# scanner-research/scannertools

Measured on AMD Instinct MI355X. Metric: 1080p frames/sec (optical-flow + histogram ops), higher is better.
Workload: dtype f32 (u8 frames in; the box filter's running sums in f64, re-anchored every 32 rows / 8 columns, column sums handed to the row pass as f32)

## Files before the change

scannertools_amd/csrc/st_context.hip:

```cpp
#include <cstring>
#include <vector>
#include <mutex>
#include <chrono>
#include <cstdlib>

#include "st_internal.h"

int st_set_error(st_ctx* ctx, int status, const char* fmt, ...) {
  char buf[512];
  va_list ap;
  va_start(ap, fmt);
  vsnprintf(buf, sizeof(buf), fmt, ap);
  va_end(ap);
  if (ctx) ctx->last_error = buf;
  return status;
}

int st_enter(st_ctx* ctx) {
  if (!ctx) return ST_ERR_INVALID;
  ST_HIP(ctx, hipSetDevice(ctx->device));
  return ST_OK;
}

namespace {
// ... 52 lines not shown
}

ST_EXPORT int st_device_count(int* count) {
  if (!count) return ST_ERR_INVALID;
  int n = 0;
  hipError_t e = hipGetDeviceCount(&n);
  if (e != hipSuccess) { *count = 0; return ST_ERR_HIP; }
  *count = n;
  return ST_OK;
}

static constexpr size_t kMinLdsBytes = 160 * 1024;

ST_EXPORT int st_ctx_create(int device_id, st_ctx** out_ctx) {
  if (!out_ctx) return ST_ERR_INVALID;
  *out_ctx = nullptr;
  int n = 0;
  if (hipGetDeviceCount(&n) != hipSuccess || device_id < 0 || device_id >= n) return ST_ERR_INVALID;
  if (hipSetDevice(device_id) != hipSuccess) return ST_ERR_HIP;
  st_ctx* c = new (std::nothrow) st_ctx();
  if (!c) return ST_ERR_OOM;
  c->device = device_id;
  if (hipStreamCreateWithFlags(&c->own_stream, hipStreamNonBlocking) != hipSuccess) {
    delete c;
    return ST_ERR_HIP;
  }
  c->stream = c->own_stream;
  if (const char* e = getenv("ST_ITER_TILE")) c->tile_mode = atoi(e);
  c->fold_gray = getenv("ST_PYR_FOLD_GRAY") != nullptr;
  if (const char* e = getenv("ST_POLY_U8")) c->poly_u8 = atoi(e) != 0;
  if (const char* e = getenv("ST_ITER_ROLES")) c->roles_mode = atoi(e);
  if (const char* e = getenv("ST_ROLES_NCW")) c->roles_ncw = atoi(e);
  if (const char* e = getenv("ST_PYR_ROLES")) c->pyr_roles = atoi(e);
  if (const char* e = getenv("ST_CONV_TILE")) c->conv_tile = atoi(e);
  if (const char* e = getenv("ST_CONCURRENT")) c->concurrency_mode = atoi(e);
  hipDeviceProp_t prop;
  if (hipGetDeviceProperties(&prop, device_id) == hipSuccess) {
    c->num_cus = prop.multiProcessorCount;
    if (prop.sharedMemPerBlock < kMinLdsBytes || strncmp(prop.gcnArchName, "gfx950", 6) != 0) {
      (void)hipStreamDestroy(c->own_stream);
      delete c;
      return ST_ERR_UNSUPPORTED;
    }
  }
  reg_add(c);
  *out_ctx = c;
  return ST_OK;
}

ST_EXPORT int st_ctx_destroy(st_ctx* ctx) {
  if (!ctx) return ST_ERR_INVALID;
  reg_remove(ctx);
  (void)hipSetDevice(ctx->device);
  (void)hipStreamSynchronize(ctx->stream);
  for (auto& t : ctx->timing) {
    for (auto e : t.starts) (void)hipEventDestroy(e);
    for (auto e : t.stops) (void)hipEventDestroy(e);
  }
  if (ctx->ws) (void)hipFree(ctx->ws);
  st_jpeg_release(ctx);
  st_netin_release(ctx);
  st_detect_release(ctx);
  if (ctx->own_stream) (void)hipStreamDestroy(ctx->own_stream);
  delete ctx;
  return ST_OK;
}
// ... 175 lines not shown
```

scannertools_amd/csrc/st_farneback.hip:

```cpp
#include <cmath>
#include <cstdlib>
#include <cstring>

#include "st_internal.h"

namespace {

constexpr int kMaxTaps = 32;
constexpr int kMaxPolyN = 7;

inline int cv_round(double v) { return (int)lrint(v); }

struct LevelGeom {
  int lh, lw, ksize;
  double sigma, scale;
};

int fb_levels(int h, int w, const st_fb_params& p) {
  int k;
  double scale = 1;
  for (k = 0; k < p.num_levels; ++k) {
    scale *= p.pyr_scale;
    if (w * scale < 32 || h * scale < 32) break;
  }
  return k;
}

LevelGeom fb_level_geom(int h, int w, const st_fb_params& p, int k) {
  LevelGeom g;
  double scale = 1;
  for (int i = 0; i < k; ++i) scale *= p.pyr_scale;
  g.scale = scale;
// ... 461 lines not shown
  float hA[KS + 1], hB[KS + 1];
#pragma unroll
  for (int j = 0; j <= KS; ++j) hA[j] = hB[j] = 0.f;
  const int ys0 = S * dy0 + OFF - r;
  const int nsrc = KS + 1 + S * (dy1 - dy0 - 1);
  int dy = dy0, until = KS + 1;
#pragma unroll 1
  for (int t = 0; t < nsrc; ++t) {
    float nA, nB;
    hrow(ys0 + t, nA, nB);
#pragma unroll
    for (int j = 0; j < KS; ++j) { hA[j] = hA[j + 1]; hB[j] = hB[j + 1]; }
    hA[KS] = nA; hB[KS] = nB;
    if (t + 1 == until) {
      until += S;
      const float b00 = pyr_colfilter<KS>(hA, a.taps), b01 = pyr_colfilter<KS>(hB, a.taps);
      const float b10 = pyr_colfilter<KS>(hA + 1, a.taps), b11 = pyr_colfilter<KS>(hB + 1, a.taps);
      float out;
      if (S == 2) {
        out = ((b00 + b01) + (b10 + b11)) * 0.25f;
      } else {
        const float r0 = b00 * 0.5f + b01 * 0.5f, r1 = b10 * 0.5f + b11 * 0.5f;
        out = r0 * 0.5f + r1 * 0.5f;
      }
      dst[(size_t)dy * a.dw + dx] = out;
      ++dy;
    }
  }
}

struct PyrFusedArgs {
  const uint8_t* gray;
  const uint8_t* const* frames;
  int cb, cg, cr, rnd, shift;
  float* img0; float* img1; float* img2; float* img3;
  int h, w, rows_per_seg;
  int strip_w;
  float k0[2], k1[2], k2[5], k3[10];
};

template <int KS>
__device__ __forceinline__ float pf_rowfilter(const float* __restrict__ b, const float* __restrict__ kh) {
  constexpr int r = KS / 2;
  if (KS == 3) return b[1] * kh[1] + (b[0] + b[2]) * kh[0];
  float v = kh[0] * b[0];
#pragma unroll
  for (int i = 1; i < KS; ++i) v += kh[i <= r ? i : KS - 1 - i] * b[i];
  return v;
}
template <int KS>
__device__ __forceinline__ float pf_colfilter(const float* __restrict__ c, const float* __restrict__ kh) {
  constexpr int r = KS / 2;
  if (KS == 3) return (c[0] + c[2]) * kh[0] + c[1] * kh[1];
  float s = kh[r] * c[r];
#pragma unroll
  for (int i = 1; i <= r; ++i) s += kh[r - i] * (c[r + i] + c[r - i]);
  return s;
}

constexpr int PF_RB = 8;
constexpr int PF_ROWDW = 260;

__device__ __forceinline__ unsigned pf_load4_border(const uint8_t* __restrict__ row, int col0, int w) {
  unsigned v = 0;
#pragma unroll 1
  for (int k = 0; k < 4; ++k) v |= (unsigned)row[d_reflect101(col0 + k, w)] << (8 * k);
// ... 154 lines not shown
        unsigned dw[6];
#pragma unroll
        for (int q = 0; q < 6; ++q) dw[q] = s[2 * u + q];
        float cb[21];
#pragma unroll
        for (int q = 0; q < 6; ++q) {
          const unsigned d = __builtin_amdgcn_alignbyte(dw[q + 1 < 6 ? q + 1 : 5], dw[q], (unsigned)half);
#pragma unroll
          for (int k = 0; k < 4; ++k)
            if (4 * q + k < 21) cb[4 * q + k] = pf_byte(d, k);
        }
        const float n3 = pf_rowfilter<19>(cb + 2, a.k3);
#pragma unroll
        for (int j = 0; j < 19; ++j) r3[j] = r3[j + 1];
        r3[19] = n3;
        if (r == 5) {
          const int dy = (y - 13) >> 3;
          if (dy >= (Y0 >> 3) && dy < (Y1 >> 3)) {
            const float c0 = pf_colfilter<19>(r3, a.k3), c1 = pf_colfilter<19>(r3 + 1, a.k3);
            const float p0 = __shfl_xor(c0, 32), p1 = __shfl_xor(c1, 32);
            if (half == 0 && live3) {
              const float q0 = c0 * 0.5f + p0 * 0.5f, q1 = c1 * 0.5f + p1 * 0.5f;
              o3[(size_t)dy * (w >> 3) + (X0 >> 3) + u] = q0 * 0.5f + q1 * 0.5f;
            }
          }
        }
      }
    }
    if (b + 1 < nb) stash(buf ^ 1);
    __syncthreads();
  }
}

template <int ROLE, bool L0 = true>
__device__ __forceinline__ void pyr_role_run(const PyrFusedArgs& a, unsigned (*srow)[PF_RB][PF_ROWDW]) {
  const int t = threadIdx.x & 255, lane = t & 63, wv = t >> 6;
  const int h = a.h, w = a.w;
  const int SW = a.strip_w;
  const int X0 = blockIdx.x * SW;
  const int Y0 = blockIdx.y * a.rows_per_seg, Y1 = min(h, Y0 + a.rows_per_seg);
  const size_t np = (size_t)h * w;
  const uint8_t* __restrict__ g = a.gray + (size_t)blockIdx.z * np;
  float* __restrict__ o0 = a.img0 + (size_t)blockIdx.z * np;
  float* __restrict__ o1 = a.img1 + (size_t)blockIdx.z * (np >> 2);
  float* __restrict__ o2 = a.img2 + (size_t)blockIdx.z * (np >> 4);
  float* __restrict__ o3 = a.img3 + (size_t)blockIdx.z * (np >> 6);
  const int u = wv * 32 + (lane & 31), half = lane >> 5;
  const bool live = 4 * t < SW && X0 + 4 * t < w;
  const bool live3 = 8 * u < SW && X0 + 8 * u < w;
  const int hq = t & 3, hrow = (t >> 2) & 7;
  const int hcol = hq < 2 ? X0 - 8 + 4 * hq : X0 + SW + 4 * (hq - 2);
  const int hidx = hq < 2 ? hq : 2 + (SW >> 2) + (hq - 2);

  unsigned pre[3], preh = 0u;
  auto fetch = [&](int ybase) {
#pragma unroll
    for (int j = 0; j < 3; ++j) {
      const int r = ROLE + 3 * j;
      if (r < PF_RB) pre[j] = pf_load4(g + (size_t)d_reflect101(ybase + r, h) * w, X0 + 4 * t, w);
    }
    if (ROLE == 0 && t < 32) preh = pf_load4(g + (size_t)d_reflect101(ybase + hrow, h) * w, hcol, w);
  };
  auto stash = [&](int buf) {
    if (4 * t < SW) {
#pragma unroll
      for (int j = 0; j < 3; ++j) {
        const int r = ROLE + 3 * j;
        if (r < PF_RB) srow[buf][r][2 + t] = pre[j];
      }
    }
    if (ROLE == 0 && t < 32) srow[buf][hrow][hidx] = preh;
  };

  float hm[4], hc[4], r1A[2][4], r1B[2][4];
  float r2A[10], r2B[10];
  float r3[20];
  if (ROLE == 0) {
#pragma unroll
    for (int j = 0; j < 4; ++j) { hm[j] = hc[j] = 0.f; r1A[0][j] = r1A[1][j] = r1B[0][j] = r1B[1][j] = 0.f; }
  } else if (ROLE == 1) {
#pragma unroll
    for (int j = 0; j < 10; ++j) r2A[j] = r2B[j] = 0.f;
  } else {
#pragma unroll
    for (int j = 0; j < 20; ++j) r3[j] = 0.f;
  }

  const int nb = (Y1 - Y0) / PF_RB + 2;
  fetch(Y0 - PF_RB);
  stash(0);
  __syncthreads();
  for (int b = 0; b < nb; ++b) {
    const int ybase = Y0 - PF_RB + b * PF_RB;
    const int buf = b & 1;
    if (b + 1 < nb) fetch(ybase + PF_RB);
#pragma unroll
    for (int r = 0; r < PF_RB; ++r) {
      const int y = ybase + r;
      const unsigned* __restrict__ s = srow[buf][r];
      if (ROLE == 0) {
        const unsigned d0 = s[t + 1], d1 = s[t + 2], d2 = s[t + 3];
        float bb[12];
#pragma unroll
        for (int k = 0; k < 4; ++k) { bb[k] = pf_byte(d0, k); bb[4 + k] = pf_byte(d1, k); bb[8 + k] = pf_byte(d2, k); }
        if (L0) {
          float hp[4];
#pragma unroll
          for (int j = 0; j < 4; ++j) hp[j] = bb[4 + j] * a.k0[1] + (bb[3 + j] + bb[5 + j]) * a.k0[0];
          const int yo = y - 1;
          if (live && yo >= Y0 && yo < Y1) {
            float4 v;
            v.x = (hm[0] + hp[0]) * a.k0[0] + hc[0] * a.k0[1];
            v.y = (hm[1] + hp[1]) * a.k0[0] + hc[1] * a.k0[1];
            v.z = (hm[2] + hp[2]) * a.k0[0] + hc[2] * a.k0[1];
            v.w = (hm[3] + hp[3]) * a.k0[0] + hc[3] * a.k0[1];
            *reinterpret_cast<float4*>(o0 + (size_t)yo * w + X0 + 4 * t) = v;
          }
#pragma unroll
          for (int j = 0; j < 4; ++j) { hm[j] = hc[j]; hc[j] = hp[j]; }
        }
        {
#pragma unroll
          for (int e = 0; e < 2; ++e) {
// ... 37 lines not shown
            const float q0 = b00 * 0.5f + b01 * 0.5f, q1 = b10 * 0.5f + b11 * 0.5f;
            o2[(size_t)dy * (w >> 2) + (X0 >> 2) + t] = q0 * 0.5f + q1 * 0.5f;
          }
        }
      } else {
        unsigned dw[6];
#pragma unroll
        for (int q = 0; q < 6; ++q) dw[q] = s[2 * u + q];
        float cb[21];
#pragma unroll
        for (int q = 0; q < 6; ++q) {
          const unsigned d = __builtin_amdgcn_alignbyte(dw[q + 1 < 6 ? q + 1 : 5], dw[q], (unsigned)half);
#pragma unroll
          for (int k = 0; k < 4; ++k)
            if (4 * q + k < 21) cb[4 * q + k] = pf_byte(d, k);
        }
        const float n3 = pf_rowfilter<19>(cb + 2, a.k3);
#pragma unroll
        for (int j = 0; j < 19; ++j) r3[j] = r3[j + 1];
        r3[19] = n3;
        if (r == 5) {
          const int dy = (y - 13) >> 3;
          if (dy >= (Y0 >> 3) && dy < (Y1 >> 3)) {
            const float c0 = pf_colfilter<19>(r3, a.k3), c1 = pf_colfilter<19>(r3 + 1, a.k3);
            const float p0 = __shfl_xor(c0, 32), p1 = __shfl_xor(c1, 32);
            if (half == 0 && live3) {
              const float q0 = c0 * 0.5f + p0 * 0.5f, q1 = c1 * 0.5f + p1 * 0.5f;
              o3[(size_t)dy * (w >> 3) + (X0 >> 3) + u] = q0 * 0.5f + q1 * 0.5f;
            }
          }
        }
      }
    }
    if (b + 1 < nb) stash(buf ^ 1);
    __syncthreads();
  }
}

template <bool L0>
__global__ __launch_bounds__(768) void k_pyr_roles(PyrFusedArgs a) {
  __shared__ unsigned srow[2][PF_RB][PF_ROWDW];
  const int role = threadIdx.x >> 8;
  if (role == 0) pyr_role_run<0, L0>(a, srow);
  else if (role == 1) pyr_role_run<1>(a, srow);
  else pyr_role_run<2>(a, srow);
}

typedef float f2u __attribute__((ext_vector_type(2), aligned(4)));
typedef float f4v16 __attribute__((ext_vector_type(4)));
__device__ __forceinline__ __amdgpu_buffer_rsrc_t st_rsrc(const void* base, size_t bytes) {
  return __builtin_amdgcn_make_buffer_rsrc(const_cast<void*>(base), 0, (int)(bytes > 0xfffffffcull ? 0xfffffffcull : bytes), 0x00020000);
}
__device__ __forceinline__ float bld1(__amdgpu_buffer_rsrc_t r, unsigned voff, unsigned soff) {
  return __builtin_bit_cast(float, __builtin_amdgcn_raw_buffer_load_b32(r, (int)voff, (int)soff, 0));
}
template <int AUX = 0>
__device__ __forceinline__ void bst1(__amdgpu_buffer_rsrc_t r, unsigned voff, unsigned soff, float v) {
  __builtin_amdgcn_raw_buffer_store_b32(__builtin_bit_cast(unsigned, v), r, (int)voff, (int)soff, AUX);
}
template <int AUX = 0>
__device__ __forceinline__ void bst4(__amdgpu_buffer_rsrc_t r, unsigned voff, float4 v) {
  typedef unsigned u4 __attribute__((ext_vector_type(4)));
  u4 q;
  q.x = __builtin_bit_cast(unsigned, v.x); q.y = __builtin_bit_cast(unsigned, v.y);
  q.z = __builtin_bit_cast(unsigned, v.z); q.w = __builtin_bit_cast(unsigned, v.w);
  __builtin_amdgcn_raw_buffer_store_b128(q, r, (int)voff, 0, AUX);
}

__device__ __forceinline__ float ldf(const float* __restrict__ base, unsigned byte_off) {
  return *reinterpret_cast<const float*>(reinterpret_cast<const char*>(base) + byte_off);
}
__device__ __forceinline__ f2u ldf2(const float* __restrict__ base, unsigned byte_off) {
  return *reinterpret_cast<const f2u*>(reinterpret_cast<const char*>(base) + byte_off);
}
__device__ __forceinline__ float4 ldf4(const float* __restrict__ base, unsigned byte_off) {
  return *reinterpret_cast<const float4*>(reinterpret_cast<const char*>(base) + byte_off);
}

// ... 832 lines not shown
  const unsigned C = gx * gy, N = C * gz;
  if (N % 8u) return;
  const unsigned L = bx + gx * (by + gy * bz), xcd = L % 8u, slot = L / 8u;
  unsigned col, pair;
  if (C % 8u == 0) {
    const unsigned cpx = C / 8u;
    col = xcd + 8u * (slot % cpx);
    pair = slot / cpx;
  } else if (8u % C == 0 && gz % (8u / C) == 0) {
    col = xcd % C;
    pair = (xcd / C) * (gz / (8u / C)) + slot;
  } else {
    return;
  }
  bx = col % gx; by = col / gx; bz = pair;
}

template <int MODE>
__global__ __launch_bounds__(B2_T, 2) void k_flow_iter3(IterArgs a) {
  typedef float f2v __attribute__((ext_vector_type(2)));
  constexpr int M = 7, W = 2 * M + 1, RB = 2;
  static_assert(W == F3_RING - 1 && F3_GROUP % RB == 0 && M <= B2_HALO, "ring of 16 = window of 15 + the entering row");
  __shared__ float Vs[F3_GROUP][5][F3_PADW];
  __shared__ float2 Fs[F3_GROUP][F3_PADW];
  const int tid = threadIdx.x;
  const int h = a.h, w = a.w;
  const int np = h * w;
  unsigned bx = blockIdx.x, by = blockIdx.y, bz = blockIdx.z;
  xcd_remap(bx, by, bz);
  const int pr = bz;
  const int x = (int)bx * B2_OUT - B2_HALO + tid;
  const int xc = d_clamp(x, 0, w - 1);
  const int y0 = by * a.rows_per_seg;
  const int y1 = min(h, y0 + a.rows_per_seg);
  const bool writer = tid >= B2_HALO && tid < B2_T - B2_HALO && x < w;
  const int vpos = f3_pos(tid);
  typedef float f4v __attribute__((ext_vector_type(4), aligned(8)));
  const bool pair_tid = tid >= B2_HALO && tid < B2_T - B2_HALO;
  const int pair_k = pair_tid ? tid - B2_HALO : 0, pair_j = pair_k % (B2_OUT / 2);
  const int pair_r0 = (pair_k / (B2_OUT / 2)) * (F3_GROUP / 2);
  const int pair_x = (int)bx * B2_OUT + 2 * pair_j;
  const int pair_pos = f3_pos(B2_HALO + 2 * pair_j);

  const float* __restrict__ R0;
  const float* __restrict__ R1;
  if (a.pairs) {
    R0 = a.R + (size_t)a.pairs[2 * pr] * 5 * (size_t)np;
    R1 = a.R + (size_t)a.pairs[2 * pr + 1] * 5 * (size_t)np;
  } else {
    R0 = a.R;
    R1 = a.R1_direct;
  }
  const float* __restrict__ fin = a.flow_in ? a.flow_in + (size_t)pr * 2 * (size_t)np : nullptr;
  const float* __restrict__ C = a.coarse ? a.coarse + (size_t)pr * 2 * (size_t)a.ch * a.cw : nullptr;
  float* fout = a.flow_ptrs ? st_gl(a.flow_ptrs[pr]) : a.flow_out + (size_t)pr * 2 * (size_t)np;
  const CoarseX cx = (MODE == FLOW_COARSE || MODE == FLOW_COARSE2) ? coarse_x(a, xc) : CoarseX{0, 1.f, 0.f, false};

  float ring[F3_RING][5];
#pragma unroll
  for (int s0 = 0; s0 < W; s0 += 3) {
    UmLoads Li[3];
    float2 f[3];
#pragma unroll
    for (int i = 0; i < 3; ++i) {
      const int yy = d_clamp(y0 - M + s0 + i, 0, h - 1);
      f[i] = iter_flow_at<MODE>(a, fin, C, cx, xc, yy);
      um_issue(R0, R1, np, h, w, xc, yy, f[i], Li[i]);
// ... 696 lines not shown
    int rows = (int)((g.lh + segs - 1) / segs);
    const int min_rows = S == 8 ? 4 : 8;
    if (rows < min_rows) rows = g.lh < min_rows ? g.lh : min_rows;
    z.rows_per_seg = rows;
    dim3 grid(bx, (g.lh + rows - 1) / rows, n);
    st_timed t(ctx, ST_K_PYR);
    if (S == 2) hipLaunchKernelGGL((k_pyr_dec<2, 3>), grid, dim3(256), 0, ctx->stream, z);
    else if (S == 4) hipLaunchKernelGGL((k_pyr_dec<4, 9>), grid, dim3(256), 0, ctx->stream, z);
    else hipLaunchKernelGGL((k_pyr_dec<8, 19>), grid, dim3(256), 0, ctx->stream, z);
    ST_HIP(ctx, hipGetLastError());
    return ST_OK;
  }
  a.mode = q.mode; a.max_rows = q.max_rows; a.max_cols = q.max_cols;
  const size_t lds = q.lds;
  if (lds > kPyrLdsMax) return st_set_error(ctx, ST_ERR_UNSUPPORTED, "farneback: pyramid tile needs %zu B of LDS", lds);
  dim3 grid((g.lw + PYR_OW - 1) / PYR_OW, (g.lh + PYR_OH - 1) / PYR_OH, n);
  st_timed t(ctx, ST_K_PYR);
  hipLaunchKernelGGL(k_pyr, grid, dim3(256), lds, ctx->stream, a);
  ST_HIP(ctx, hipGetLastError());
  return ST_OK;
}

bool pyr_fused_ok(int h, int w, const st_fb_params& p) {
  if (fb_levels(h, w, p) != 3 || (h & 7) || (w & 7)) return false;
  static const int ks[4] = {3, 3, 9, 19};
  for (int k = 0; k <= 3; ++k) {
    const LevelGeom g = fb_level_geom(h, w, p, k);
    if (g.lh != (h >> k) || g.lw != (w >> k) || g.ksize != ks[k]) return false;
  }
  return true;
}

int launch_pyr_fused(st_ctx* ctx, const uint8_t* gray, const uint8_t* const* frames, int n, int h, int w,
                     const st_fb_params& p, float* const imgs[4], bool skip0 = false) {
  PyrFusedArgs a;
  memset(&a, 0, sizeof(a));
  a.gray = gray; a.frames = frames;
  if (p.gray_bits == 14) { a.cb = 1868; a.cg = 9617; a.cr = 4899; } else { a.cb = 3735; a.cg = 19235; a.cr = 9798; }
  a.shift = p.gray_bits; a.rnd = 1 << (p.gray_bits - 1);
  a.img0 = imgs[0]; a.img1 = imgs[1]; a.img2 = imgs[2]; a.img3 = imgs[3];
  a.h = h; a.w = w;
  float* taps[4] = {a.k0, a.k1, a.k2, a.k3};
  for (int k = 0; k <= 3; ++k) {
    const LevelGeom g = fb_level_geom(h, w, p, k);
    float full[kMaxTaps];
    gaussian_kernel(g.ksize, g.sigma, full);
    for (int i = 0; i <= g.ksize / 2; ++i) {
      if (full[i] != full[g.ksize - 1 - i]) return st_set_error(ctx, ST_ERR_UNSUPPORTED, "pyr: asymmetric Gaussian taps");
      taps[k][i] = full[i];
    }
  }
  const int strips = (w + 1023) / 1024;
  a.strip_w = ((w + strips - 1) / strips + 7) / 8 * 8;
  const bool roles_on = gray && ctx->pyr_roles != 0;
  long long segs = ((long long)ctx->num_cus * (roles_on ? 14 : 8) + (long long)strips * n - 1) / ((long long)strips * n);
  int rows = (int)((h + segs - 1) / segs);
  rows = (rows + 7) / 8 * 8;
  const int min_rows = (long long)strips * n * ((h + 63) / 64) >= 2LL * ctx->num_cus ? 64 : 16;
  if (rows < min_rows) rows = h < min_rows ? h : min_rows;
  a.rows_per_seg = rows;
  st_timed t(ctx, ST_K_PYR);
  const int roles_env = ctx->pyr_roles;
  const bool roles = gray && roles_env != 0;
  if (skip0 && !roles) return st_set_error(ctx, ST_ERR_INVALID, "pyr: level 0 can only be left out of the role-split kernel");
  if (roles && skip0) hipLaunchKernelGGL(k_pyr_roles<false>, dim3(strips, (h + rows - 1) / rows, n), dim3(768), 0, ctx->stream, a);
  else if (roles) hipLaunchKernelGGL(k_pyr_roles<true>, dim3(strips, (h + rows - 1) / rows, n), dim3(768), 0, ctx->stream, a);
  else if (gray) hipLaunchKernelGGL(k_pyr_fused<false>, dim3(strips, (h + rows - 1) / rows, n), dim3(256), 0, ctx->stream, a);
  else hipLaunchKernelGGL(k_pyr_fused<true>, dim3(strips, (h + rows - 1) / rows, n), dim3(256), 0, ctx->stream, a);
  ST_HIP(ctx, hipGetLastError());
  return ST_OK;
}

static bool polyexp_frame_fits(int h, int w) { return (unsigned long long)h * (unsigned long long)w <= (1ull << 26); }

int launch_polyexp(st_ctx* ctx, const float* img, int n, int h, int w, int poly_n, double poly_sigma, float* R,
                   const uint8_t* gray = nullptr) {
  if (!polyexp_frame_fits(h, w)) return st_set_error(ctx, ST_ERR_UNSUPPORTED, "polyexp: frames above 64 M pixels are not supported");
  PolyArgs a;
  a.img = img; a.gray = gray; a.R = R; a.h = h; a.w = w;
  poly_prepare(poly_n, poly_sigma, &a.c);
  const int strips = (w + PE_OUT - 1) / PE_OUT;
  a.rows_per_seg = polyexp_rows(ctx, h, strips, n, poly_n);
  dim3 grid(strips, (h + a.rows_per_seg - 1) / a.rows_per_seg, n);
  st_timed t(ctx, ST_K_POLYEXP);
  if (gray && w < 8) return st_set_error(ctx, ST_ERR_INVALID, "polyexp: the gray-source instance needs rows of at least 8 pixels");
  if (gray && poly_n == 5) hipLaunchKernelGGL(k_polyexp_u8<5>, grid, dim3(256), 0, ctx->stream, a);
  else if (gray) hipLaunchKernelGGL(k_polyexp_u8<7>, grid, dim3(256), 0, ctx->stream, a);
  else if (poly_n == 5) hipLaunchKernelGGL(k_polyexp<5>, grid, dim3(256), 0, ctx->stream, a);
  else hipLaunchKernelGGL(k_polyexp<7>, grid, dim3(256), 0, ctx->stream, a);
  ST_HIP(ctx, hipGetLastError());
  return ST_OK;
}

int launch_polyexp_ml(st_ctx* ctx, float* const* imgs, const LevelGeom* geom, float* const* R, const int* ks, int nk, int n,
                      int poly_n, double poly_sigma) {
  if (nk < 1 || nk > 4) return st_set_error(ctx, ST_ERR_INVALID, "polyexp: bad level list");
  PolyArgsML a;
  memset(&a, 0, sizeof(a));
// ... 22 lines not shown
  int bx = (int)((np + 255) / 256);
  if (bx > 4096) bx = 4096;
  st_timed t(ctx, ST_K_UPDATE_MATRICES);
  hipLaunchKernelGGL(k_update_matrices, dim3(bx, n_pairs), dim3(256), 0, ctx->stream, a);
  ST_HIP(ctx, hipGetLastError());
  return ST_OK;
}

int launch_blur(st_ctx* ctx, BlurArgs a, int n_pairs) {
  if (a.m == 7) {
    const int strips = (a.w + B2_OUT - 1) / B2_OUT;
    long long segs = ((long long)ctx->num_cus * 4 + (long long)strips - 1) / ((long long)strips);
    int rows = (int)((a.h + segs - 1) / segs);
    rows = (rows + 14) / 15 * 15;
    if (rows < 15) rows = 15;
    if (rows > 135 && a.h > 135) rows = 135;
    a.rows_per_seg = rows;
    dim3 grid(strips, (a.h + rows - 1) / rows, n_pairs);
    st_timed t(ctx, ST_K_BLUR_UPDATE);
    hipLaunchKernelGGL((k_blur_update_v2<7>), grid, dim3(B2_T), 0, ctx->stream, a);
    ST_HIP(ctx, hipGetLastError());
    return ST_OK;
  }
  const int strips = (a.w + (BLUR_T - 2 * a.m) - 1) / (BLUR_T - 2 * a.m);
  a.rows_per_seg = rows_per_segment(ctx, a.h, strips, 1, 2 * a.m + 1);
  dim3 grid(strips, (a.h + a.rows_per_seg - 1) / a.rows_per_seg, n_pairs);
  st_timed t(ctx, ST_K_BLUR_UPDATE);
  hipLaunchKernelGGL(k_blur_update, grid, dim3(BLUR_T), 0, ctx->stream, a);
  ST_HIP(ctx, hipGetLastError());
  return ST_OK;
}

int launch_flow_iter(st_ctx* ctx, IterArgs a, int n_pairs) {
  constexpr long long kTilePx = 600000;
  const bool tile = ctx->tile_mode == 1 || (ctx->tile_mode != 0 && (long long)n_pairs * a.h * a.w <= kTilePx);
  if (tile && (a.h + FT_T - 1) / FT_T <= 65535) {
    dim3 grid((a.w + FT_T - 1) / FT_T, (a.h + FT_T - 1) / FT_T, n_pairs);
    st_timed t(ctx, ST_K_BLUR_UPDATE);
    if (a.coarse) hipLaunchKernelGGL((k_flow_iter_tile<FLOW_COARSE>), grid, dim3(FT_NT), 0, ctx->stream, a);
    else if (a.flow_in) hipLaunchKernelGGL((k_flow_iter_tile<FLOW_FIELD>), grid, dim3(FT_NT), 0, ctx->stream, a);
    else hipLaunchKernelGGL((k_flow_iter_tile<FLOW_ZERO>), grid, dim3(FT_NT), 0, ctx->stream, a);
    ST_HIP(ctx, hipGetLastError());
    return ST_OK;
  }
  const int strips = (a.w + B2_OUT - 1) / B2_OUT;
  const long long resident = (long long)ctx->num_cus * 2;
  const int periods = (a.h + F3_ANCHOR - 1) / F3_ANCHOR;
  int rows = periods * F3_ANCHOR;
  long long rounds3 = 1, wgs3 = 1;
  double best = 1e300;
  for (int segs = 1; segs <= periods; ++segs) {
    const int r = (periods + segs - 1) / segs * F3_ANCHOR;
    const long long nseg = (a.h + r - 1) / r;
    const long long wgs = (long long)strips * n_pairs * nseg;
    const long long rounds = (wgs + resident - 1) / resident;
    const double cost = (double)rounds * (r + 15);
    if (cost < best * 0.999) { best = cost; rows = r; rounds3 = rounds; wgs3 = wgs; }
  }
  const int roles_env = ctx->roles_mode == -1 && ctx->flow_concurrent ? 0 : ctx->roles_mode;
  const int roles_ncw = ctx->roles_ncw;
  const long long roles_limit = a.coarse ? resident * 62 / 100 : resident * 95 / 100;
  if (roles_env == 1 || (roles_env != 0 && rounds3 == 1 && wgs3 < roles_limit)) {
    int best_ncw = 0, best_out = 0, best_rows = 0;
    double bestr = 1e300;
    for (int ncw = 5; ncw >= 4; --ncw) {
      if (roles_ncw && ncw != roles_ncw) continue;
      const int outmax = 64 * ncw - 2 * B2_HALO;
      const int rstrips = (a.w + outmax - 1) / outmax;
      const int out_w = ((a.w + rstrips - 1) / rstrips + 7) / 8 * 8;
      for (int segs = 1; segs <= periods; ++segs) {
        const int r = (periods + segs - 1) / segs * F3_ANCHOR;
        const long long nseg = (a.h + r - 1) / r;
        const long long wgs = (long long)rstrips * n_pairs * nseg;
        const long long rounds = (wgs + ctx->num_cus - 1) / ctx->num_cus;
        const double cost = (double)rounds * (r + 16 + 3 * FR_G) * (ncw == 5 ? 1.3 : 1.0);
        if (cost < bestr * 0.999) { bestr = cost; best_ncw = ncw; best_out = out_w; best_rows = r; }
      }
    }
    if (best_ncw) {
      a.rows_per_seg = best_rows;
      a.out_w = best_out;
      const int rstrips = (a.w + best_out - 1) / best_out;
      dim3 grid(rstrips, (a.h + best_rows - 1) / best_rows, n_pairs);
      st_timed t(ctx, ST_K_BLUR_UPDATE);
      const int mode = a.coarse ? (a.h == 2 * a.ch ? FLOW_COARSE2 : FLOW_COARSE) : (a.flow_in ? FLOW_FIELD : FLOW_ZERO);
      if (best_ncw == 5) {
        const dim3 blk(FrGeom<5>::THREADS);
        if (mode == FLOW_COARSE2) hipLaunchKernelGGL((k_flow_iter_roles<5, FLOW_COARSE2>), grid, blk, 0, ctx->stream, a);
        else if (mode == FLOW_COARSE) hipLaunchKernelGGL((k_flow_iter_roles<5, FLOW_COARSE>), grid, blk, 0, ctx->stream, a);
        else if (mode == FLOW_FIELD) hipLaunchKernelGGL((k_flow_iter_roles<5, FLOW_FIELD>), grid, blk, 0, ctx->stream, a);
        else hipLaunchKernelGGL((k_flow_iter_roles<5, FLOW_ZERO>), grid, blk, 0, ctx->stream, a);
      } else {
        const dim3 blk(FrGeom<4>::THREADS);
        if (mode == FLOW_COARSE2) hipLaunchKernelGGL((k_flow_iter_roles<4, FLOW_COARSE2>), grid, blk, 0, ctx->stream, a);
        else if (mode == FLOW_COARSE) hipLaunchKernelGGL((k_flow_iter_roles<4, FLOW_COARSE>), grid, blk, 0, ctx->stream, a);
        else if (mode == FLOW_FIELD) hipLaunchKernelGGL((k_flow_iter_roles<4, FLOW_FIELD>), grid, blk, 0, ctx->stream, a);
        else hipLaunchKernelGGL((k_flow_iter_roles<4, FLOW_ZERO>), grid, blk, 0, ctx->stream, a);
      }
      ST_HIP(ctx, hipGetLastError());
      return ST_OK;
    }
  }
  a.rows_per_seg = rows;
  dim3 grid(strips, (a.h + rows - 1) / rows, n_pairs);
  st_timed t(ctx, ST_K_BLUR_UPDATE);
  const int mode = a.coarse ? (a.h == 2 * a.ch ? FLOW_COARSE2 : FLOW_COARSE) : (a.flow_in ? FLOW_FIELD : FLOW_ZERO);
  if (mode == FLOW_COARSE2) hipLaunchKernelGGL((k_flow_iter3<FLOW_COARSE2>), grid, dim3(B2_T), 0, ctx->stream, a);
  else if (mode == FLOW_COARSE) hipLaunchKernelGGL((k_flow_iter3<FLOW_COARSE>), grid, dim3(B2_T), 0, ctx->stream, a);
  else if (mode == FLOW_FIELD) hipLaunchKernelGGL((k_flow_iter3<FLOW_FIELD>), grid, dim3(B2_T), 0, ctx->stream, a);
  else hipLaunchKernelGGL((k_flow_iter3<FLOW_ZERO>), grid, dim3(B2_T), 0, ctx->stream, a);
  ST_HIP(ctx, hipGetLastError());
  return ST_OK;
}

bool fused_path(int h, int w, const st_fb_params& p) {
  if (p.win_size != 15) return false;
  const int levels = fb_levels(h, w, p);
  for (int k = 0; k <= levels; ++k) {
    LevelGeom g = fb_level_geom(h, w, p, k);
    if (g.lh < 2 || g.lw < 2) return false;
  }
  return true;
}

size_t pass_bytes(int h, int w, const st_fb_params& p, int nf, int npairs) {
  const int levels = fb_levels(h, w, p);
  size_t np0 = (size_t)h * w;
  size_t maxCoarse = 0;
  for (int k = 0; k <= levels; ++k) {
    LevelGeom g = fb_level_geom(h, w, p, k);
    size_t npk = (size_t)g.lh * g.lw;
    if (k >= 1 && npk > maxCoarse) maxCoarse = npk;
  }
  size_t b = 0;
  b += st_align_up(np0 * nf);
  b += st_align_up(sizeof(float) * np0 * nf);
  if (pyr_fused_ok(h, w, p))
    for (int k = 1; k <= 3; ++k) b += st_align_up(sizeof(float) * (np0 >> (2 * k)) * nf);
  for (int k = 0; k <= levels; ++k) {
    LevelGeom g = fb_level_geom(h, w, p, k);
    b += st_align_up(sizeof(float) * 5 * (size_t)g.lh * g.lw * nf);
  }
  b += 2 * st_align_up(sizeof(float) * (fused_path(h, w, p) ? 2 : 5) * np0 * npairs);
// ... 24 lines not shown
    size_t npk = (size_t)geom[k].lh * geom[k].lw;
    if (k >= 1 && npk > maxCoarse) maxCoarse = npk;
    R[k] = (float*)st_ws_alloc(ctx, sizeof(float) * 5 * npk * nf);
  }
  float* M[2];
  const bool fused = fused_path(h, w, p);
  M[0] = (float*)st_ws_alloc(ctx, sizeof(float) * (fused ? 2 : 5) * np0 * npairs);
  M[1] = (float*)st_ws_alloc(ctx, sizeof(float) * (fused ? 2 : 5) * np0 * npairs);
  float* cflow[2];
  cflow[0] = (float*)st_ws_alloc(ctx, sizeof(float) * 2 * maxCoarse * npairs);
  cflow[1] = (float*)st_ws_alloc(ctx, sizeof(float) * 2 * maxCoarse * npairs);
  const uint8_t** d_frames = (const uint8_t**)st_ws_alloc(ctx, sizeof(void*) * nf);
  int* d_pairs = (int*)st_ws_alloc(ctx, sizeof(int) * 2 * npairs);
  float** d_outs = (float**)st_ws_alloc(ctx, sizeof(void*) * npairs);
  if (!gray || !img || !M[0] || !M[1] || !cflow[0] || !cflow[1] || !d_frames || !d_pairs || !d_outs || !R[levels])
    return st_set_error(ctx, ST_ERR_OOM, "farneback: scratch plan exhausted");
  TablesArg ta;
  const bool small_tables = nf <= kTabMax && npairs <= kTabMax;
  if (small_tables) {
    memset(&ta, 0, sizeof(ta));
    ta.d_frames = d_frames; ta.d_outs = d_outs; ta.d_pairs = d_pairs; ta.nf = nf; ta.npairs = npairs;
    for (int i = 0; i < nf; ++i) ta.frames[i] = frames[i];
    for (int i = 0; i < npairs; ++i) { ta.outs[i] = outs[i]; ta.pairs[2 * i] = pairs[2 * i]; ta.pairs[2 * i + 1] = pairs[2 * i + 1]; }
    static_assert(kTabMax <= 64, "one thread per table entry");
  } else {
    ST_HIP(ctx, hipMemcpyAsync(d_frames, frames, sizeof(void*) * nf, hipMemcpyHostToDevice, ctx->stream));
    ST_HIP(ctx, hipMemcpyAsync(d_pairs, pairs, sizeof(int) * 2 * npairs, hipMemcpyHostToDevice, ctx->stream));
    ST_HIP(ctx, hipMemcpyAsync(d_outs, outs, sizeof(void*) * npairs, hipMemcpyHostToDevice, ctx->stream));
  }

  bool aligned4 = true;
  for (int i = 0; i < nf; ++i) aligned4 = aligned4 && ((uintptr_t)frames[i] & 3) == 0;
  const bool pyr_rgb = pyr1 && aligned4 && ctx->fold_gray;
  if (!pyr_rgb) {
    ST_TRY(launch_gray(ctx, d_frames, nf, h, w, p.gray_bits, gray, aligned4, small_tables ? &ta : nullptr));
  } else if (small_tables) {
    hipLaunchKernelGGL(k_set_tables, dim3(1), dim3(64), 0, ctx->stream, ta);
    ST_HIP(ctx, hipGetLastError());
  }
  const bool single = pyr1 && levels >= 1 && levels <= 3 && npairs <= 16;
  const bool poly_u8 = pyr1 && !pyr_rgb && !single && ctx->poly_u8 && ctx->pyr_roles != 0 && geom[0].ksize == 3 && geom[0].sigma <= 0 &&
                       geom[0].lh == h && geom[0].lw == w && w >= 8;
  if (pyr1) ST_TRY(launch_pyr_fused(ctx, pyr_rgb ? nullptr : gray, d_frames, nf, h, w, p, imgs, poly_u8));
  if (single) {
    int ks[4], nk = 0;
    for (int k = 0; k <= levels; ++k) ks[nk++] = k;
    ST_TRY(launch_polyexp_ml(ctx, imgs, geom.data(), R.data(), ks, nk, nf, p.poly_n, p.poly_sigma));
  } else {
    for (int k = levels; k >= 0; --k) {
      if (!pyr1) ST_TRY(launch_pyr(ctx, gray, nf, h, w, geom[k], img));
      ST_TRY(launch_polyexp(ctx, pyr1 ? imgs[k] : img, nf, geom[k].lh, geom[k].lw, p.poly_n, p.poly_sigma, R[k],
                            k == 0 && poly_u8 ? gray : nullptr));
    }
  }
  if (fused) {
    float* fbuf[2] = {M[0], M[1]};
    int cur = 0;
    for (int k = levels; k >= 0; --k) {
      const int lh = geom[k].lh, lw = geom[k].lw;
      for (int it = 0; it < p.num_iters; ++it) {
        const bool last = it == p.num_iters - 1;
        IterArgs q;
        memset(&q, 0, sizeof(q));
        q.R = R[k]; q.pairs = d_pairs; q.h = lh; q.w = lw;
        q.scale = 1. / ((double)p.win_size * p.win_size);
        if (it == 0) {
          if (k < levels) {
            q.coarse = cflow[cur];
            q.ch = geom[k + 1].lh; q.cw = geom[k + 1].lw;
            q.scale_x = 1. / ((double)lw / q.cw);
            q.scale_y = 1. / ((double)lh / q.ch);
            q.mul = (float)(1. / p.pyr_scale);
          }
        } else {
          q.flow_in = fbuf[(it - 1) & 1];
        }
// ... 215 lines not shown
```

scannertools_amd/csrc/st_internal.h:

```cpp
#ifndef ST_INTERNAL_H_
#define ST_INTERNAL_H_

#include <hip/hip_runtime.h>

#include <atomic>
#include <cstdarg>
#include <cstdio>
#include <string>
#include <vector>

#include "scannertools_hip.h"

#define ST_EXPORT extern "C" __attribute__((visibility("default")))

struct st_timing_slot {
  std::vector<hipEvent_t> starts, stops;
  size_t used = 0;
  int launches = 0;
  double total_ms = 0.0;
};

struct st_ctx {
  int device = 0;
  hipStream_t own_stream = nullptr;
  hipStream_t stream = nullptr;
  int tile_mode = -1;
  bool poly_u8 = true;
  bool fold_gray = false;
  int roles_mode = -1, roles_ncw = 0, pyr_roles = -1;
  int conv_tile = -1;
  std::atomic<bool> flow_busy{false};
  std::atomic<long long> flow_enter_ns{0};
  bool flow_concurrent = false;
  int concurrency_mode = -1;
  void* ws = nullptr;
  size_t ws_bytes = 0;
  size_t ws_limit = (size_t)64 << 30;
  size_t ws_off = 0;
  unsigned timing_mask = 0;
  st_timing_slot timing[ST_K_COUNT];
  std::string last_error;
  int num_cus = 256;
  struct st_jpeg_state* jpeg = nullptr;
  struct st_netin_state* netin = nullptr;
  struct st_detect_state* detect = nullptr;
};
void st_jpeg_release(st_ctx* ctx);
void st_netin_release(st_ctx* ctx);
void st_detect_release(st_ctx* ctx);

int st_set_error(st_ctx* ctx, int status, const char* fmt, ...);

#define ST_HIP(ctx, expr)                                                                   \
  do {                                                                                      \
    hipError_t _e = (expr);                                                                 \
    if (_e != hipSuccess)                                                                   \
      return st_set_error((ctx), ST_ERR_HIP, "%s failed: %s (%s:%d)", #expr,                \
                          hipGetErrorString(_e), __FILE__, __LINE__);                       \
  } while (0)

#define ST_TRY(expr)              \
  do {                            \
// ... 124 lines not shown
```

Measured before the change: 9804.

## Fold RGB-to-gray conversion into role-split pyramid kernel and retune flow segments

Adds an RGB-source variant of the role-split pyramid kernel. It reads packed RGB frames with nontemporal loads, converts them to gray in registers, and writes the gray image out as a side product, so the separate gray-conversion launch is skipped. It is on by default through pyr_roles_rgb. The change also adds a segment-count search for the k_flow_iter3 grid, where the last segment absorbs the remainder rows, and moves flow-iteration timing onto hipExtLaunchKernelGGL events instead of a scoped timer. The risks are extra register pressure from the raw RGB buffers and partial-row gray writes being correct only when live is set.

```diff
diff --git a/scannertools_amd/csrc/st_context.hip b/scannertools_amd/csrc/st_context.hip
--- a/scannertools_amd/csrc/st_context.hip
+++ b/scannertools_amd/csrc/st_context.hip
@@ -108,6 +108,7 @@
   if (const char* e = getenv("ST_ITER_ROLES")) c->roles_mode = atoi(e);
   if (const char* e = getenv("ST_ROLES_NCW")) c->roles_ncw = atoi(e);
   if (const char* e = getenv("ST_PYR_ROLES")) c->pyr_roles = atoi(e);
+  if (const char* e = getenv("ST_PYR_ROLES_RGB")) c->pyr_roles_rgb = atoi(e) != 0;
   if (const char* e = getenv("ST_CONV_TILE")) c->conv_tile = atoi(e);
   if (const char* e = getenv("ST_CONCURRENT")) c->concurrency_mode = atoi(e);
   hipDeviceProp_t prop;
diff --git a/scannertools_amd/csrc/st_farneback.hip b/scannertools_amd/csrc/st_farneback.hip
--- a/scannertools_amd/csrc/st_farneback.hip
+++ b/scannertools_amd/csrc/st_farneback.hip
@@ -1,3 +1,5 @@
+#include <hip/hip_ext.h>
+
 #include <cmath>
 #include <cstdlib>
 #include <cstring>
@@ -525,6 +527,7 @@
 struct PyrFusedArgs {
   const uint8_t* gray;
   const uint8_t* const* frames;
+  uint8_t* gray_out;
   int cb, cg, cr, rnd, shift;
   float* img0; float* img1; float* img2; float* img3;
   int h, w, rows_per_seg;
@@ -745,7 +748,26 @@
   }
 }
 
-template <int ROLE, bool L0 = true>
+typedef unsigned pf_u3nt __attribute__((ext_vector_type(3), aligned(4)));
+__device__ __forceinline__ pf_u3nt pf_fetch_rgb(const uint8_t* __restrict__ row, int col0, int w, const PyrFusedArgs& a) {
+  if (col0 >= 0 && col0 + 3 < w) return __builtin_nontemporal_load(reinterpret_cast<const pf_u3nt*>(row + 3 * col0));
+  pf_u3nt v = {0u, 0u, 0u};
+  if (col0 >= w + 8 || col0 < -8) return v;
+#pragma unroll
+  for (int k = 0; k < 4; ++k) v.x |= pf_gray1(row + 3 * d_reflect101(col0 + k, w), a) << (8 * k);
+  return v;
+}
+__device__ __forceinline__ unsigned pf_gray_of(pf_u3nt v, bool inside, const PyrFusedArgs& a) {
+  if (!inside) return v.x;
+  const unsigned w0 = v.x, w1 = v.y, w2 = v.z;
+  const int g0 = (int)((w0 & 0xff) * a.cb + ((w0 >> 8) & 0xff) * a.cg + ((w0 >> 16) & 0xff) * a.cr + a.rnd) >> a.shift;
+  const int g1 = (int)((w0 >> 24) * a.cb + (w1 & 0xff) * a.cg + ((w1 >> 8) & 0xff) * a.cr + a.rnd) >> a.shift;
+  const int g2 = (int)(((w1 >> 16) & 0xff) * a.cb + (w1 >> 24) * a.cg + (w2 & 0xff) * a.cr + a.rnd) >> a.shift;
+  const int g3 = (int)(((w2 >> 8) & 0xff) * a.cb + ((w2 >> 16) & 0xff) * a.cg + (w2 >> 24) * a.cr + a.rnd) >> a.shift;
+  return (unsigned)g0 | ((unsigned)g1 << 8) | ((unsigned)g2 << 16) | ((unsigned)g3 << 24);
+}
+
+template <int ROLE, bool L0 = true, bool RGB = false>
 __device__ __forceinline__ void pyr_role_run(const PyrFusedArgs& a, unsigned (*srow)[PF_RB][PF_ROWDW]) {
   const int t = threadIdx.x & 255, lane = t & 63, wv = t >> 6;
   const int h = a.h, w = a.w;
@@ -753,7 +775,8 @@
   const int X0 = blockIdx.x * SW;
   const int Y0 = blockIdx.y * a.rows_per_seg, Y1 = min(h, Y0 + a.rows_per_seg);
   const size_t np = (size_t)h * w;
-  const uint8_t* __restrict__ g = a.gray + (size_t)blockIdx.z * np;
+  const uint8_t* __restrict__ g = RGB ? st_gl(a.frames[blockIdx.z]) : a.gray + (size_t)blockIdx.z * np;
+  const int gw = RGB ? 3 * w : w;
   float* __restrict__ o0 = a.img0 + (size_t)blockIdx.z * np;
   float* __restrict__ o1 = a.img1 + (size_t)blockIdx.z * (np >> 2);
   float* __restrict__ o2 = a.img2 + (size_t)blockIdx.z * (np >> 4);
@@ -764,25 +787,39 @@
   const int hq = t & 3, hrow = (t >> 2) & 7;
   const int hcol = hq < 2 ? X0 - 8 + 4 * hq : X0 + SW + 4 * (hq - 2);
   const int hidx = hq < 2 ? hq : 2 + (SW >> 2) + (hq - 2);
+  const bool in_t = X0 + 4 * t + 3 < w, in_h = hcol >= 0 && hcol + 3 < w;
+  uint8_t* __restrict__ gout = RGB ? a.gray_out + (size_t)blockIdx.z * np : nullptr;
 
   unsigned pre[3], preh = 0u;
+  pf_u3nt raw[3] = {{0u, 0u, 0u}, {0u, 0u, 0u}, {0u, 0u, 0u}}, rawh = {0u, 0u, 0u};
   auto fetch = [&](int ybase) {
 #pragma unroll
     for (int j = 0; j < 3; ++j) {
       const int r = ROLE + 3 * j;
-      if (r < PF_RB) pre[j] = pf_load4(g + (size_t)d_reflect101(ybase + r, h) * w, X0 + 4 * t, w);
-    }
-    if (ROLE == 0 && t < 32) preh = pf_load4(g + (size_t)d_reflect101(ybase + hrow, h) * w, hcol, w);
+      if (r < PF_RB) {
+        if (RGB) { if (4 * t < SW) raw[j] = pf_fetch_rgb(g + (size_t)d_reflect101(ybase + r, h) * gw, X0 + 4 * t, w, a); }
+        else pre[j] = pf_load4(g + (size_t)d_reflect101(ybase + r, h) * gw, X0 + 4 * t, w);
+      }
+    }
+    if (ROLE == 0 && t < 32) {
+      if (RGB) rawh = pf_fetch_rgb(g + (size_t)d_reflect101(ybase + hrow, h) * gw, hcol, w, a);
+      else preh = pf_load4(g + (size_t)d_reflect101(ybase + hrow, h) * gw, hcol, w);
+    }
   };
-  auto stash = [&](int buf) {
+  auto stash = [&](int buf, int ybase) {
+    const bool own = RGB && ybase >= Y0 && ybase < Y1;
     if (4 * t < SW) {
 #pragma unroll
       for (int j = 0; j < 3; ++j) {
         const int r = ROLE + 3 * j;
-        if (r < PF_RB) srow[buf][r][2 + t] = pre[j];
+        if (r < PF_RB) {
+          const unsigned v = RGB ? pf_gray_of(raw[j], in_t, a) : pre[j];
+          srow[buf][r][2 + t] = v;
+          if (RGB && own && live) *reinterpret_cast<unsigned*>(gout + (size_t)(ybase + r) * w + X0 + 4 * t) = v;
+        }
       }
     }
-    if (ROLE == 0 && t < 32) srow[buf][hrow][hidx] = preh;
+    if (ROLE == 0 && t < 32) srow[buf][hrow][hidx] = RGB ? pf_gray_of(rawh, in_h, a) : preh;
   };
 
   float hm[4], hc[4], r1A[2][4], r1B[2][4];
@@ -801,7 +838,7 @@
 
   const int nb = (Y1 - Y0) / PF_RB + 2;
   fetch(Y0 - PF_RB);
-  stash(0);
+  stash(0, Y0 - PF_RB);
   __syncthreads();
   for (int b = 0; b < nb; ++b) {
     const int ybase = Y0 - PF_RB + b * PF_RB;
@@ -905,18 +942,19 @@
         }
       }
     }
-    if (b + 1 < nb) stash(buf ^ 1);
+    if (b + 1 < nb) stash(buf ^ 1, ybase + PF_RB);
     __syncthreads();
   }
 }
 
-template <bool L0>
+template <bool L0, bool RGB = false>
 __global__ __launch_bounds__(768) void k_pyr_roles(PyrFusedArgs a) {
+  static_assert(!(L0 && RGB), "the RGB-source instance leaves level 0 to k_polyexp_u8");
   __shared__ unsigned srow[2][PF_RB][PF_ROWDW];
   const int role = threadIdx.x >> 8;
-  if (role == 0) pyr_role_run<0, L0>(a, srow);
-  else if (role == 1) pyr_role_run<1>(a, srow);
-  else pyr_role_run<2>(a, srow);
+  if (role == 0) pyr_role_run<0, L0, RGB>(a, srow);
+  else if (role == 1) pyr_role_run<1, true, RGB>(a, srow);
+  else pyr_role_run<2, true, RGB>(a, srow);
 }
 
 typedef float f2u __attribute__((ext_vector_type(2), aligned(4)));
@@ -1815,7 +1853,7 @@
   const int x = (int)bx * B2_OUT - B2_HALO + tid;
   const int xc = d_clamp(x, 0, w - 1);
   const int y0 = by * a.rows_per_seg;
-  const int y1 = min(h, y0 + a.rows_per_seg);
+  const int y1 = by + 1 == gridDim.y ? h : min(h, y0 + a.rows_per_seg);
   const bool writer = tid >= B2_HALO && tid < B2_T - B2_HALO && x < w;
   const int vpos = f3_pos(tid);
   typedef float f4v __attribute__((ext_vector_type(4), aligned(8)));
@@ -2578,10 +2616,11 @@
 }
 
 int launch_pyr_fused(st_ctx* ctx, const uint8_t* gray, const uint8_t* const* frames, int n, int h, int w,
-                     const st_fb_params& p, float* const imgs[4], bool skip0 = false) {
+                     const st_fb_params& p, float* const imgs[4], bool skip0 = false, bool gray_out = false) {
   PyrFusedArgs a;
   memset(&a, 0, sizeof(a));
   a.gray = gray; a.frames = frames;
+  if (gray_out) a.gray_out = const_cast<uint8_t*>(gray);
   if (p.gray_bits == 14) { a.cb = 1868; a.cg = 9617; a.cr = 4899; } else { a.cb = 3735; a.cg = 19235; a.cr = 9798; }
   a.shift = p.gray_bits; a.rnd = 1 << (p.gray_bits - 1);
   a.img0 = imgs[0]; a.img1 = imgs[1]; a.img2 = imgs[2]; a.img3 = imgs[3];
@@ -2609,7 +2648,9 @@
   const int roles_env = ctx->pyr_roles;
   const bool roles = gray && roles_env != 0;
   if (skip0 && !roles) return st_set_error(ctx, ST_ERR_INVALID, "pyr: level 0 can only be left out of the role-split kernel");
-  if (roles && skip0) hipLaunchKernelGGL(k_pyr_roles<false>, dim3(strips, (h + rows - 1) / rows, n), dim3(768), 0, ctx->stream, a);
+  if (gray_out && !(skip0 && frames)) return st_set_error(ctx, ST_ERR_INVALID, "pyr: the RGB-source role-split kernel leaves level 0 out");
+  if (gray_out) hipLaunchKernelGGL((k_pyr_roles<false, true>), dim3(strips, (h + rows - 1) / rows, n), dim3(768), 0, ctx->stream, a);
+  else if (roles && skip0) hipLaunchKernelGGL(k_pyr_roles<false>, dim3(strips, (h + rows - 1) / rows, n), dim3(768), 0, ctx->stream, a);
   else if (roles) hipLaunchKernelGGL(k_pyr_roles<true>, dim3(strips, (h + rows - 1) / rows, n), dim3(768), 0, ctx->stream, a);
   else if (gray) hipLaunchKernelGGL(k_pyr_fused<false>, dim3(strips, (h + rows - 1) / rows, n), dim3(256), 0, ctx->stream, a);
   else hipLaunchKernelGGL(k_pyr_fused<true>, dim3(strips, (h + rows - 1) / rows, n), dim3(256), 0, ctx->stream, a);
@@ -2698,14 +2739,15 @@
 }
 
 int launch_flow_iter(st_ctx* ctx, IterArgs a, int n_pairs) {
+  hipEvent_t e0, e1;
   constexpr long long kTilePx = 600000;
   const bool tile = ctx->tile_mode == 1 || (ctx->tile_mode != 0 && (long long)n_pairs * a.h * a.w <= kTilePx);
   if (tile && (a.h + FT_T - 1) / FT_T <= 65535) {
     dim3 grid((a.w + FT_T - 1) / FT_T, (a.h + FT_T - 1) / FT_T, n_pairs);
-    st_timed t(ctx, ST_K_BLUR_UPDATE);
-    if (a.coarse) hipLaunchKernelGGL((k_flow_iter_tile<FLOW_COARSE>), grid, dim3(FT_NT), 0, ctx->stream, a);
-    else if (a.flow_in) hipLaunchKernelGGL((k_flow_iter_tile<FLOW_FIELD>), grid, dim3(FT_NT), 0, ctx->stream, a);
-    else hipLaunchKernelGGL((k_flow_iter_tile<FLOW_ZERO>), grid, dim3(FT_NT), 0, ctx->stream, a);
+    ST_TRY(st_time_dispatch(ctx, ST_K_BLUR_UPDATE, &e0, &e1));
+    if (a.coarse) hipExtLaunchKernelGGL((k_flow_iter_tile<FLOW_COARSE>), grid, dim3(FT_NT), 0, ctx->stream, e0, e1, 0, a);
+    else if (a.flow_in) hipExtLaunchKernelGGL((k_flow_iter_tile<FLOW_FIELD>), grid, dim3(FT_NT), 0, ctx->stream, e0, e1, 0, a);
+    else hipExtLaunchKernelGGL((k_flow_iter_tile<FLOW_ZERO>), grid, dim3(FT_NT), 0, ctx->stream, e0, e1, 0, a);
     ST_HIP(ctx, hipGetLastError());
     return ST_OK;
   }
@@ -2748,33 +2790,43 @@
       a.out_w = best_out;
       const int rstrips = (a.w + best_out - 1) / best_out;
       dim3 grid(rstrips, (a.h + best_rows - 1) / best_rows, n_pairs);
-      st_timed t(ctx, ST_K_BLUR_UPDATE);
+      ST_TRY(st_time_dispatch(ctx, ST_K_BLUR_UPDATE, &e0, &e1));
       const int mode = a.coarse ? (a.h == 2 * a.ch ? FLOW_COARSE2 : FLOW_COARSE) : (a.flow_in ? FLOW_FIELD : FLOW_ZERO);
       if (best_ncw == 5) {
         const dim3 blk(FrGeom<5>::THREADS);
-        if (mode == FLOW_COARSE2) hipLaunchKernelGGL((k_flow_iter_roles<5, FLOW_COARSE2>), grid, blk, 0, ctx->stream, a);
-        else if (mode == FLOW_COARSE) hipLaunchKernelGGL((k_flow_iter_roles<5, FLOW_COARSE>), grid, blk, 0, ctx->stream, a);
-        else if (mode == FLOW_FIELD) hipLaunchKernelGGL((k_flow_iter_roles<5, FLOW_FIELD>), grid, blk, 0, ctx->stream, a);
-        else hipLaunchKernelGGL((k_flow_iter_roles<5, FLOW_ZERO>), grid, blk, 0, ctx->stream, a);
+        if (mode == FLOW_COARSE2) hipExtLaunchKernelGGL((k_flow_iter_roles<5, FLOW_COARSE2>), grid, blk, 0, ctx->stream, e0, e1, 0, a);
+        else if (mode == FLOW_COARSE) hipExtLaunchKernelGGL((k_flow_iter_roles<5, FLOW_COARSE>), grid, blk, 0, ctx->stream, e0, e1, 0, a);
+        else if (mode == FLOW_FIELD) hipExtLaunchKernelGGL((k_flow_iter_roles<5, FLOW_FIELD>), grid, blk, 0, ctx->stream, e0, e1, 0, a);
+        else hipExtLaunchKernelGGL((k_flow_iter_roles<5, FLOW_ZERO>), grid, blk, 0, ctx->stream, e0, e1, 0, a);
       } else {
         const dim3 blk(FrGeom<4>::THREADS);
-        if (mode == FLOW_COARSE2) hipLaunchKernelGGL((k_flow_iter_roles<4, FLOW_COARSE2>), grid, blk, 0, ctx->stream, a);
-        else if (mode == FLOW_COARSE) hipLaunchKernelGGL((k_flow_iter_roles<4, FLOW_COARSE>), grid, blk, 0, ctx->stream, a);
-        else if (mode == FLOW_FIELD) hipLaunchKernelGGL((k_flow_iter_roles<4, FLOW_FIELD>), grid, blk, 0, ctx->stream, a);
-        else hipLaunchKernelGGL((k_flow_iter_roles<4, FLOW_ZERO>), grid, blk, 0, ctx->stream, a);
+        if (mode == FLOW_COARSE2) hipExtLaunchKernelGGL((k_flow_iter_roles<4, FLOW_COARSE2>), grid, blk, 0, ctx->stream, e0, e1, 0, a);
+        else if (mode == FLOW_COARSE) hipExtLaunchKernelGGL((k_flow_iter_roles<4, FLOW_COARSE>), grid, blk, 0, ctx->stream, e0, e1, 0, a);
+        else if (mode == FLOW_FIELD) hipExtLaunchKernelGGL((k_flow_iter_roles<4, FLOW_FIELD>), grid, blk, 0, ctx->stream, e0, e1, 0, a);
+        else hipExtLaunchKernelGGL((k_flow_iter_roles<4, FLOW_ZERO>), grid, blk, 0, ctx->stream, e0, e1, 0, a);
       }
       ST_HIP(ctx, hipGetLastError());
       return ST_OK;
     }
   }
+  int nseg3 = (a.h + rows - 1) / rows;
+  for (int segs = 1; segs <= periods; ++segs) {
+    const int r = periods / segs * F3_ANCHOR;
+    if (r < F3_ANCHOR) break;
+    const int last = a.h - (segs - 1) * r;
+    const long long wgs = (long long)strips * n_pairs * segs;
+    const long long rounds = (wgs + resident - 1) / resident;
+    const double cost = (double)rounds * ((r > last ? r : last) + 15);
+    if (cost < best * 0.999) { best = cost; rows = r; nseg3 = segs; }
+  }
   a.rows_per_seg = rows;
-  dim3 grid(strips, (a.h + rows - 1) / rows, n_pairs);
-  st_timed t(ctx, ST_K_BLUR_UPDATE);
+  dim3 grid(strips, nseg3, n_pairs);
+  ST_TRY(st_time_dispatch(ctx, ST_K_BLUR_UPDATE, &e0, &e1));
   const int mode = a.coarse ? (a.h == 2 * a.ch ? FLOW_COARSE2 : FLOW_COARSE) : (a.flow_in ? FLOW_FIELD : FLOW_ZERO);
-  if (mode == FLOW_COARSE2) hipLaunchKernelGGL((k_flow_iter3<FLOW_COARSE2>), grid, dim3(B2_T), 0, ctx->stream, a);
-  else if (mode == FLOW_COARSE) hipLaunchKernelGGL((k_flow_iter3<FLOW_COARSE>), grid, dim3(B2_T), 0, ctx->stream, a);
-  else if (mode == FLOW_FIELD) hipLaunchKernelGGL((k_flow_iter3<FLOW_FIELD>), grid, dim3(B2_T), 0, ctx->stream, a);
-  else hipLaunchKernelGGL((k_flow_iter3<FLOW_ZERO>), grid, dim3(B2_T), 0, ctx->stream, a);
+  if (mode == FLOW_COARSE2) hipExtLaunchKernelGGL((k_flow_iter3<FLOW_COARSE2>), grid, dim3(B2_T), 0, ctx->stream, e0, e1, 0, a);
+  else if (mode == FLOW_COARSE) hipExtLaunchKernelGGL((k_flow_iter3<FLOW_COARSE>), grid, dim3(B2_T), 0, ctx->stream, e0, e1, 0, a);
+  else if (mode == FLOW_FIELD) hipExtLaunchKernelGGL((k_flow_iter3<FLOW_FIELD>), grid, dim3(B2_T), 0, ctx->stream, e0, e1, 0, a);
+  else hipExtLaunchKernelGGL((k_flow_iter3<FLOW_ZERO>), grid, dim3(B2_T), 0, ctx->stream, e0, e1, 0, a);
   ST_HIP(ctx, hipGetLastError());
   return ST_OK;
 }
@@ -2865,16 +2917,17 @@
   bool aligned4 = true;
   for (int i = 0; i < nf; ++i) aligned4 = aligned4 && ((uintptr_t)frames[i] & 3) == 0;
   const bool pyr_rgb = pyr1 && aligned4 && ctx->fold_gray;
-  if (!pyr_rgb) {
+  const bool single = pyr1 && levels >= 1 && levels <= 3 && npairs <= 16;
+  const bool poly_u8 = pyr1 && !pyr_rgb && !single && ctx->poly_u8 && ctx->pyr_roles != 0 && geom[0].ksize == 3 && geom[0].sigma <= 0 &&
+                       geom[0].lh == h && geom[0].lw == w && w >= 8;
+  const bool roles_rgb = poly_u8 && aligned4 && ctx->pyr_roles_rgb;
+  if (!pyr_rgb && !roles_rgb) {
     ST_TRY(launch_gray(ctx, d_frames, nf, h, w, p.gray_bits, gray, aligned4, small_tables ? &ta : nullptr));
   } else if (small_tables) {
     hipLaunchKernelGGL(k_set_tables, dim3(1), dim3(64), 0, ctx->stream, ta);
     ST_HIP(ctx, hipGetLastError());
   }
-  const bool single = pyr1 && levels >= 1 && levels <= 3 && npairs <= 16;
-  const bool poly_u8 = pyr1 && !pyr_rgb && !single && ctx->poly_u8 && ctx->pyr_roles != 0 && geom[0].ksize == 3 && geom[0].sigma <= 0 &&
-                       geom[0].lh == h && geom[0].lw == w && w >= 8;
-  if (pyr1) ST_TRY(launch_pyr_fused(ctx, pyr_rgb ? nullptr : gray, d_frames, nf, h, w, p, imgs, poly_u8));
+  if (pyr1) ST_TRY(launch_pyr_fused(ctx, pyr_rgb ? nullptr : gray, d_frames, nf, h, w, p, imgs, poly_u8, roles_rgb));
   if (single) {
     int ks[4], nk = 0;
     for (int k = 0; k <= levels; ++k) ks[nk++] = k;
diff --git a/scannertools_amd/csrc/st_internal.h b/scannertools_amd/csrc/st_internal.h
--- a/scannertools_amd/csrc/st_internal.h
+++ b/scannertools_amd/csrc/st_internal.h
@@ -28,6 +28,7 @@
   bool poly_u8 = true;
   bool fold_gray = false;
   int roles_mode = -1, roles_ncw = 0, pyr_roles = -1;
+  bool pyr_roles_rgb = true;
   int conv_tile = -1;
   std::atomic<bool> flow_busy{false};
   std::atomic<long long> flow_enter_ns{0};
```

After: 9972 (median of 6 runs). 1.7% higher.
